# posgraph/coupe.DVSG

Hardware: AMD Instinct MI355X
Metric: stabilized frames/sec (1280x720 RGB) (higher is better)
Workload: dtype f32

## Files before the change

### coupe/dvsg_amd/csrc/cnn_kernels.h

```cpp
#pragma once
#include <type_traits>

#include "common.h"

namespace dvsg {

enum Precision { kF32 = 0, kF16 = 1, kF32S = 2, kF32X = 3 };
inline size_t elem_size(int prec) { return prec == kF16 ? 2 : 4; }

struct ConvGemm {
  int prec;
  const void *x;
  const void *wt;
  const float *bias;
  const void *res;
  void *y;
  int B, H, W, Cin, Ho, Wo, Cout;
  int ksize, stride, pad;
  int res_H, res_W, res_stride;
  int relu;
  int ldx = 0, res_ld = 0, relu_from = -1;
  const void *wt_packed = nullptr;
  const void *wt_packed_a = nullptr;
  const void *wt_packed_h = nullptr;
// ... 12 lines not shown
extern int g_last_conv_kernel[kConvKernelFields];
inline void record_conv_kernel(int family, int a0 = -1, int a1 = -1, int a2 = -1, int a3 = -1, int wsrc = -1) {
  const int rec[kConvKernelFields] = {family, a0, a1, a2, a3, wsrc};
  for (int i = 0; i < kConvKernelFields; ++i) g_last_conv_kernel[i] = rec[i];
}
inline void reset_conv_kernel() { record_conv_kernel(-1); }
template <typename F>
void with_relu_res(bool relu, int res, F &&f) {
  auto with_res = [&](auto relu_c) {
    if (res == 0) f(relu_c, std::integral_constant<int, 0>{});
    else if (res == 1) f(relu_c, std::integral_constant<int, 1>{});
    else f(relu_c, std::integral_constant<int, 2>{});
  };
  if (relu) with_res(std::true_type{});
  else with_res(std::false_type{});
}
inline size_t x3_packed_bytes(int rows, int K) { return (size_t)rows * K * 6; }
int launch_pack_x3(const float *wt, void *out, int rows, int K, hipStream_t s);
int launch_conv_wide16(const ConvGemm &p, hipStream_t s);
size_t wide16_packed_bytes(int rows, int Cin, int ksize);
int launch_pack_wide16(const void *wt, void *out, int rows, int Cin, int ksize, int order, hipStream_t s);
int launch_zero_tickets(int *tickets, size_t n, hipStream_t s);
struct ConvFused {
  const float *x;
  const float *wt2;
  const float *bias2;
  const float *wt3;
  const float *bias3;
  const float *res;
  float *y;
  int B, H, W, Cin, Ho, Wo, Cout;
  int stride;
  int res_H, res_W, res_stride;
  const float *sc_x = nullptr;
  const float *sc_wt = nullptr;
  const float *sc_bias = nullptr;
  int sc_cin = 0;
  int pieces = 0;
  int f16 = 0;
  int x3 = 0;
};
int launch_conv3x3_1x1_x3(const ConvFused &p, hipStream_t s);
bool conv_fusable(int prec, int Cin, int Cmid, int Cout, int ksize);
int launch_conv3x3_1x1(const ConvFused &p, hipStream_t s);

constexpr int kConv1Cin = 21;
constexpr int kConv1K = 7 * kConv1Cin;
constexpr int kConv1Kpad = 148;
constexpr int kConv1Ld = 150;
constexpr int kConv1LdH = 168;
constexpr int kConv1X3Ld = 88;
constexpr int kConv1X3StageElems = 3 * 64 * kConv1X3Ld;
constexpr int kRootMaxFrames = 16;
constexpr int rootconv_pitch(int cin) { return cin | 1; }
constexpr int rootconv_kpad(int cin) { return (7 * rootconv_pitch(cin) + 3) & ~3; }
constexpr int rootconv_ld(int cin) { return rootconv_kpad(cin) + 2; }
constexpr int kRootKernelFields = 9;
enum RootKernelField { kRootConv1 = 0, kRootNW, kRootTO, kRootSRC, kRootBands, kRootQuads, kRootMaxpool, kRootAvgpool,
                       kRootDenseChunks };
extern int g_last_root_kernel[kRootKernelFields];
inline void reset_root_kernel() {
  for (int i = 0; i < kRootKernelFields; ++i) g_last_root_kernel[i] = -1;
}
inline void record_conv1_kernel(int family, int nw, int to, int src, int bands = -1, int quads = -1) {
  const int rec[6] = {family, nw, to, src, bands, quads};
  for (int i = 0; i < 6; ++i) g_last_root_kernel[i] = rec[i];
}
enum Conv1SrcKind { kSrcWindow = 0, kSrcRingF32 = 1, kSrcRingU8 = 2 };
constexpr int kSrcAligned = 1;
constexpr int kSrcKindShift = 1;
constexpr int kSrcMasked = 8;
constexpr int conv1_src(int kind, bool aligned, bool masked) {
  return (kind << kSrcKindShift) | (aligned ? kSrcAligned : 0) | (masked ? kSrcMasked : 0);
}
struct Conv1Src {
  const void *base;
  const int *table;
  int n_pool;
  const float *mask = nullptr;
};
int launch_conv1(int out_prec, const Conv1Src &src, int src_kind, const float *wt1, const void *wt1h, const void *wt1s,
                 const void *wt1x, const float *bias, void *y, int B, int H, int W, int Ho, int Wo, int cin, hipStream_t s);
int prepare_rootconv();

int launch_maxpool(int prec, const void *x, void *y, int B, int H, int W, int C, int Ho, int Wo, int pad_top,
                   int pad_left, hipStream_t s);

constexpr int kPoolSplits = 8;
int launch_avgpool_partial(int prec, const void *x, float *part, int B, int HW, int C, hipStream_t s);

int launch_f16_to_f32(const void *x, float *y, size_t n, hipStream_t s);
int launch_p_to_f32(const void *x, float *y, size_t n, hipStream_t s);
int launch_f32_to_p(const float *x, void *y, size_t n, hipStream_t s);

constexpr int kDenseSplits = 8;
int launch_dense(const float *xin, int s_in, const float *bias_in, float scale_in, int lrelu_in,
                 const float *W, float *out_part, int B, int K, int N, hipStream_t s);
int launch_dense_finalize(const float *part, int s_in, float scale, const float *bias, float *out, int B,
                          int N, hipStream_t s);

}
```

### coupe/dvsg_amd/csrc/conv1_pool.hip

```cpp
#include <cstdint>
#include <type_traits>
#include <utility>

#include "cnn_device.h"
#include "cnn_kernels.h"

namespace dvsg {
namespace {

constexpr int C1_TILE = 128;
constexpr int C1_SEG_PAD = 5488;
constexpr int C1_WELEMS = 64 * kConv1Ld;
constexpr int C1_LDC = 68;

template <int NT, int GROUPS, bool ALIGNED, bool MASKED = false>
struct Conv1Row {
  static constexpr bool kRing = false;
  typedef float floatx4_u __attribute__((ext_vector_type(4), aligned(4)));
  floatx4 nmean[GROUPS];
  long idx[GROUPS];
  unsigned col_ok, full;
  bool fast;
  struct Data {
    floatx4 reg[GROUPS];
// ... 376 lines not shown
#pragma unroll
    for (int q = 0; q < 16; ++q) acc[mi][q] = acc2[mi][q] = 0.f;

#ifdef DVSG_STAMPS
  unsigned long long st[8] = {0, 0, 0, 0, 0, 0, 0, 0};
  const unsigned long long t_begin = C1_STAMP(), r_begin = __builtin_amdgcn_s_memrealtime();
#endif
  load_stage(0);
#ifdef DVSG_STAMPS
  st[0] = C1_STAMP() - t_begin;
#endif
  for (int kh = 0; kh < 7; ++kh) {
#ifdef DVSG_STAMPS
    const unsigned long long s0 = C1_STAMP();
    __syncthreads();
    const unsigned long long s1 = C1_STAMP();
    store_stage();
    const unsigned long long s2 = C1_STAMP();
    __syncthreads();
    const unsigned long long s3 = C1_STAMP();
    if (kh + 1 < 7) load_stage(kh + 1);
    const unsigned long long s4 = C1_STAMP();
    st[1] += s1 - s0;
    st[2] += s2 - s1;
    st[3] += s3 - s2;
    st[4] += s4 - s3;
#else
    __syncthreads();
    store_stage();
    __syncthreads();
    if (kh + 1 < 7) load_stage(kh + 1);
#endif
    __builtin_amdgcn_sched_barrier(0);
    const float *a0 = in_s + 2 * kConv1Cin * (wm * 32 * MI + r) + 2 * h;
    const float *bp = w_s + (wn * 32 + r) * kConv1Ld + 2 * h;
    constexpr int STEPS = kConv1Kpad / 4, PAIRS = (STEPS + 1) / 2;
    float2 va[2][2][MI], vb[2][2];
    auto read_pair = [&](int slot, int g) __attribute__((always_inline)) {
#pragma unroll
      for (int j = 0; j < 2; ++j) {
        if (2 * g + j >= STEPS) break;
#pragma unroll
        for (int mi = 0; mi < MI; ++mi)
          va[slot][j][mi] = *reinterpret_cast<const float2 *>(a0 + mi * (2 * kConv1Cin * 32) + 4 * (2 * g + j));
        vb[slot][j] = *reinterpret_cast<const float2 *>(bp + 4 * (2 * g + j));
      }
    };
    read_pair(0, 0);
#pragma unroll
    for (int g = 0; g < PAIRS; ++g) {
      if (g + 1 < PAIRS) read_pair((g + 1) & 1, g + 1);
      __builtin_amdgcn_sched_barrier(0);
#pragma unroll
      for (int j = 0; j < 2; ++j) {
        if (2 * g + j >= STEPS) break;
#pragma unroll
        for (int mi = 0; mi < MI; ++mi) acc[mi] = mfma32(va[g & 1][j][mi].x, vb[g & 1][j].x, acc[mi]);
#pragma unroll
        for (int mi = 0; mi < MI; ++mi) acc2[mi] = mfma32(va[g & 1][j][mi].y, vb[g & 1][j].y, acc2[mi]);
      }
      __builtin_amdgcn_sched_barrier(0);
    }
  }

#ifdef DVSG_STAMPS
  const unsigned long long t_loop_end = C1_STAMP();
#endif
  float *Cs = w_s;
  __syncthreads();
#pragma unroll
  for (int mi = 0; mi < MI; ++mi)
    C1_TILE_PUT(Cs, wm * 32 * MI + mi * 32, wn * 32, acc[mi][q] + acc2[mi][q]);
  __syncthreads();
  TO *yrow = y + (((size_t)b * Ho + ho) * Wo + wo0) * 64 + 4 * (tid & 15);
  conv1_tile_out<NT / 16>(Cs, conv1_tile_bias(bias, tid), tid, wo0, Wo,
                          [&](int row, float4 v) __attribute__((always_inline)) { store4(yrow + (size_t)row * 64, v); });
#ifdef DVSG_STAMPS
  if (tid == 0 && blockIdx.x < 65536) {
    unsigned long long *o = g_c1_stamps + (size_t)blockIdx.x * 8;
    const unsigned long long t_end = C1_STAMP();
    o[0] = st[0]; o[1] = st[1]; o[2] = st[2]; o[3] = st[3]; o[4] = st[4];
    o[5] = t_loop_end - t_begin;
    o[6] = t_end - t_begin;
    o[7] = __builtin_amdgcn_s_memrealtime() - r_begin;
  }
#endif
}

struct PPieces {};

constexpr int rootconv_seg(int cin) { return C1_RING_PX * rootconv_pitch(cin) + 4; }
constexpr int rootconv_wstage(int cin) { return 64 * rootconv_ld(cin) > C1_TILE * C1_LDC ? 64 * rootconv_ld(cin) : C1_TILE * C1_LDC; }
constexpr size_t rootconv_lds_bytes(int cin) { return sizeof(float) * (size_t)(rootconv_wstage(cin) + rootconv_seg(cin)); }
static_assert(rootconv_lds_bytes(3 * kRootMaxFrames) <= 160 * 1024, "the largest window must fit one workgroup's LDS");

template <typename TO, int SRC>
__global__ __launch_bounds__(256)
void rootconv_kernel(const Conv1Src src, const float *__restrict__ wt1, const float *__restrict__ bias, void *__restrict__ y,
                     int H, int W, int Ho, int Wo, int wtiles, int cin) {
  constexpr int NT = 256, MI = 2;
  constexpr int kKind = SRC >> kSrcKindShift & 3;
  constexpr bool kMasked = (SRC & kSrcMasked) != 0;
  static_assert(SRC >= 0 && SRC < 16 && kKind <= kSrcRingU8, "no such conv1 source");
  extern __shared__ __attribute__((aligned(16))) float rc_lds[];
  const int S = cin / 3, pitch = rootconv_pitch(cin), ldw = rootconv_ld(cin), steps = rootconv_kpad(cin) / 4;
  const int welems = 64 * ldw, seg = rootconv_seg(cin);
  float *w_s = rc_lds;
  float *in_s = rc_lds + rootconv_wstage(cin);
  const int tid = threadIdx.x;
  const int lane = tid & 63, wave = tid >> 6;
  const int wm = wave >> 1, wn = wave & 1;
  const int r = lane & 31, h = lane >> 5;

  const Conv1Tile tile = conv1_tile(wtiles, Ho);
  const int b = tile.b, ho = tile.ho, wo0 = tile.wo0;

  for (int e = tid; e < seg; e += NT) in_s[e] = 0.f;

  const float *mplane = nullptr;
  if constexpr (kMasked) mplane = src.mask + (size_t)b * H * W;
  const int items = C1_RING_PX * S;
  auto stage = [&](int kh) __attribute__((always_inline)) {
    const int hi = 2 * ho + kh - 3;
    const bool row_ok = hi >= 0 && hi < H;
    for (int q = tid; q < items; q += NT) {
      const int f = q / C1_RING_PX, p = q - f * C1_RING_PX;
      const int col = 2 * wo0 - 3 + p;
      float a[3] = {0.f, 0.f, 0.f};
      if (row_ok && col >= 0 && col < W) {
        const size_t px = (size_t)hi * W + col;
        float m = 1.0f;
        bool masked = false;
        if constexpr (kMasked) {
          masked = f < S - 1;
          if (masked) m = mplane[px];
        }
        float s3[3];
        if constexpr (kKind == kSrcWindow) {
          const float *x = static_cast<const float *>(src.base) + ((size_t)b * H * W + px) * cin + 3 * f;
#pragma unroll
          for (int j = 0; j < 3; ++j) s3[j] = masked ? (x[j] * m) * 255.0f : x[j] * 255.0f;
        } else {
          const int fi = src.table[b * S + f];
          const bool frame_ok = fi >= 0 && fi < src.n_pool;
          const size_t e0 = ((size_t)(frame_ok ? fi : 0) * H * W + px) * 3;
          if constexpr (kKind == kSrcRingU8) {
            const uint8_t *x = static_cast<const uint8_t *>(src.base) + e0;
#pragma unroll
            for (int j = 0; j < 3; ++j) {
              const float v = (float)x[j];
              if (masked) {
                const float q0 = v * (1.0f / 255.0f);
                const float xf = __builtin_fmaf(__builtin_fmaf(-q0, 255.0f, v), 1.0f / 255.0f, q0);
                s3[j] = (xf * m) * 255.0f;
              } else {
                s3[j] = v;
              }
            }
          } else {
            const float *x = static_cast<const float *>(src.base) + e0;
#pragma unroll
            for (int j = 0; j < 3; ++j) s3[j] = masked ? (x[j] * m) * 255.0f : x[j] * 255.0f;
          }
          if (!frame_ok) s3[0] = s3[1] = s3[2] = 0.f;
        }
#pragma unroll
// ... 926 lines not shown
    constexpr bool PIPE = SRC < 2;
    Frag fr[PIPE ? 2 : 1];
    if (PIPE) read_a(fr[0], 0);
#pragma unroll
    for (int t = 0; t < 5; ++t) {
      bf16x8 bw[3][2];
#pragma unroll
      for (int p = 0; p < 3; ++p)
#pragma unroll
        for (int ni = 0; ni < 2; ++ni)
          bw[p][ni] = *reinterpret_cast<const bf16x8 *>(b0 + (p * 64 + ni * 32) * kConv1X3Ld + 16 * t);
      if (PIPE) {
        if (t + 1 < 5) read_a(fr[(t + 1) & 1], t + 1);
      } else {
        read_a(fr[0], t);
      }
      __builtin_amdgcn_sched_barrier(0);
      const Frag &f = fr[PIPE ? (t & 1) : 0];
#define DVSG_C1X_TERM(C, PA, PB) \
  _Pragma("unroll") for (int ni = 0; ni < 2; ++ni) C[ni] = __builtin_amdgcn_mfma_f32_32x32x16_bf16(f.a[PA].v, bw[PB][ni], C[ni], 0, 0, 0)
      DVSG_C1X_TERM(accs, 2, 0);
      DVSG_C1X_TERM(accs, 0, 2);
      DVSG_C1X_TERM(accs, 1, 1);
      DVSG_C1X_TERM(accs, 1, 0);
      DVSG_C1X_TERM(accs, 0, 1);
      DVSG_C1X_TERM(acc, 0, 0);
#undef DVSG_C1X_TERM
      __builtin_amdgcn_sched_barrier(0);
    }
  }

  float *Cs = reinterpret_cast<float *>(w_s);
  __syncthreads();
#pragma unroll
  for (int ni = 0; ni < 2; ++ni)
    C1_TILE_PUT(Cs, wave * 32, ni * 32, acc[ni][q] + accs[ni][q]);
  __syncthreads();
  const int col4 = tid & 15;
  conv1_tile_out<16>(Cs, conv1_tile_bias(bias, tid), tid, wo0, Wo, [&](int row, float4 v) __attribute__((always_inline)) {
    store4(y + (((size_t)b * Ho + ho) * Wo + wo0 + row) * 64 + 4 * col4, v);
  });
}

__global__ __launch_bounds__(256) void maxpool_p_kernel(const void *__restrict__ x, void *__restrict__ y, int H, int W,
                                                       int C4, int Ho, int Wo, int pad_top, int pad_left, size_t total) {
  const size_t e = (size_t)xcd_remap(blockIdx.x, gridDim.x) * 256 + threadIdx.x;
  if (e >= total) return;
  const int c4 = (int)(e % C4);
  size_t t = e / C4;
  const int wo = (int)(t % Wo);
  t /= Wo;
  const int ho = (int)(t % Ho);
  const size_t b = t / Ho;
  float4 m = make_float4(-INFINITY, -INFINITY, -INFINITY, -INFINITY);
#pragma unroll
  for (int i = 0; i < 3; ++i) {
    const int hi = 2 * ho - pad_top + i;
    if (hi < 0 || hi >= H) continue;
#pragma unroll
    for (int j = 0; j < 3; ++j) {
      const int wi = 2 * wo - pad_left + j;
      if (wi < 0 || wi >= W) continue;
      const float4 v = load4_p(x, (((b * H + hi) * W + wi) * C4 + c4) * 4);
      m.x = fmaxf(m.x, v.x);
      m.y = fmaxf(m.y, v.y);
      m.z = fmaxf(m.z, v.z);
      m.w = fmaxf(m.w, v.w);
    }
  }
  store4_p(y, e * 4, m);
}

int march_bands(int B, int Ho, int wtiles, int *quads_per_band) {
  const int quads = (Ho + C1M_QUAD - 1) / C1M_QUAD;
  const long cols = (long)B * wtiles;
  for (int qpb = 8; qpb >= 4; --qpb) {
    const int bands = (quads + qpb - 1) / qpb;
    if (cols * bands >= 3 * 256) {
      if (quads_per_band) *quads_per_band = qpb;
      return bands;
    }
  }
  return 0;
}

template <int S>
using SrcC = std::integral_constant<int, S>;
template <bool MASKED_TOO, typename F>
bool with_conv1_src(int src, F &&f) {
  auto is = [&](auto c) { return src == c && (f(c), true); };
  if (is(SrcC<conv1_src(kSrcWindow, false, false)>{}) || is(SrcC<conv1_src(kSrcWindow, true, false)>{}) ||
      is(SrcC<conv1_src(kSrcRingF32, false, false)>{}) || is(SrcC<conv1_src(kSrcRingF32, true, false)>{}) ||
      is(SrcC<conv1_src(kSrcRingU8, false, false)>{}) || is(SrcC<conv1_src(kSrcRingU8, true, false)>{}))
    return true;
  if constexpr (MASKED_TOO)
    return is(SrcC<conv1_src(kSrcWindow, false, true)>{}) || is(SrcC<conv1_src(kSrcWindow, true, true)>{}) ||
           is(SrcC<conv1_src(kSrcRingF32, false, true)>{}) || is(SrcC<conv1_src(kSrcRingF32, true, true)>{}) ||
           is(SrcC<conv1_src(kSrcRingU8, false, true)>{}) || is(SrcC<conv1_src(kSrcRingU8, true, true)>{});
  return false;
}

}

int g_last_root_kernel[kRootKernelFields] = {-1, -1, -1, -1, -1, -1, -1, -1, -1};

int launch_conv1(int out_prec, const Conv1Src &src, int src_kind, const float *wt1, const void *wt1h, const void *wt1s,
                 const void *wt1x, const float *bias, void *y, int B, int H, int W, int Ho, int Wo, int cin, hipStream_t s) {
  DVSG_REQUIRE(cin % 3 == 0 && cin >= 3 && cin <= 3 * kRootMaxFrames, "conv1: %d input channels", cin);
  const int wtiles = ceil_div(Wo, C1_TILE);
  const long blocks = (long)wtiles * Ho * B;
  DVSG_REQUIRE(blocks > 0 && blocks < (1L << 31), "conv1: grid of %ld workgroups out of range", blocks);
  DVSG_REQUIRE((long)W * cin < (1L << 31), "conv1: input row too long");
  DVSG_REQUIRE(src_kind == kSrcWindow || (src.table && src.n_pool > 0), "conv1: a frame ring needs its index table");
  const double in_bytes = src_kind == kSrcRingU8 ? 1.0 : 4.0;
  ProfScope prof(kClsConv1, s, 2.0 * (double)B * Ho * Wo * 64 * 49 * cin,
                 in_bytes * (double)B * H * W * cin + (double)elem_size(out_prec) * B * Ho * Wo * 64);
  const dim3 grid((unsigned)blocks);
  const bool aligned = W % 4 == 0 && reinterpret_cast<uintptr_t>(src.base) % (src_kind == kSrcRingU8 ? 4 : 16) == 0;
  const int SRC = conv1_src(src_kind, aligned, src.mask != nullptr);
  if (cin != kConv1Cin) {
    DVSG_REQUIRE(wt1, "conv1: no float32 weight image");
    const int to = out_prec == kF16 ? 1 : (out_prec == kF32S ? 2 : 0);
    const size_t lds = rootconv_lds_bytes(cin);
    const bool known = with_conv1_src<true>(SRC, [&](auto src_c) {
      constexpr int S = decltype(src_c)::value;
      record_conv1_kernel(6, 4, to, S);
      if (to == 1)
        hipLaunchKernelGGL((rootconv_kernel<_Float16, S>), grid, dim3(256), lds, s, src, wt1, bias, y, H, W, Ho, Wo, wtiles, cin);
      else if (to == 2)
        hipLaunchKernelGGL((rootconv_kernel<PPieces, S>), grid, dim3(256), lds, s, src, wt1, bias, y, H, W, Ho, Wo, wtiles, cin);
      else
        hipLaunchKernelGGL((rootconv_kernel<float, S>), grid, dim3(256), lds, s, src, wt1, bias, y, H, W, Ho, Wo, wtiles, cin);
    });
    DVSG_REQUIRE(known, "conv1: no kernel for source %d", SRC);
    return check_launch("rootconv_kernel");
  }
  if (out_prec == kF32S && !wt1s) return fail(DVSG_ERR_UNSUPPORTED, "conv1: the f32s precision needs the piece weights");
  if (out_prec == kF32X && !wt1x) return fail(DVSG_ERR_UNSUPPORTED, "conv1: the f32x3 precision needs the bfloat16 piece weights");
  const int variant = g_opt.conv1_variant;
  bool legal = true;
  if (out_prec == kF32X) {
    legal = with_conv1_src<true>(SRC, [&](auto src_c) {
      constexpr int S = decltype(src_c)::value;
      record_conv1_kernel(5, -1, -1, S);
      hipLaunchKernelGGL((conv1_x3_kernel<S>), grid, dim3(256), 0, s, src, static_cast<const unsigned short *>(wt1x), bias,
                         static_cast<float *>(y), H, W, Ho, Wo, wtiles);
    });
  } else if (out_prec == kF32S) {
    legal = with_conv1_src<true>(SRC, [&](auto src_c) {
      constexpr int S = decltype(src_c)::value;
      record_conv1_kernel(4, -1, 0, S);
      hipLaunchKernelGGL((conv1_split_kernel<float, S>), grid, dim3(256), 0, s, src, static_cast<const _Float16 *>(wt1s), bias,
                         static_cast<float *>(y), H, W, Ho, Wo, wtiles);
    });
  } else if (out_prec == kF16 && wt1h && variant == 3 && !src.mask) {
    legal = with_conv1_src<false>(SRC, [&](auto src_c) {
      constexpr int S = decltype(src_c)::value;
      record_conv1_kernel(1, -1, 1, S);
      hipLaunchKernelGGL((conv1_f16_kernel<_Float16, S>), grid, dim3(256), 0, s, src, static_cast<const _Float16 *>(wt1h), bias,
                         static_cast<_Float16 *>(y), H, W, Ho, Wo, wtiles);
    });
  } else if (out_prec == kF16 && wt1h && variant != 2 && variant != 4 && !src.mask &&
             (variant == 5 || march_bands(B, Ho, wtiles, nullptr) > 0)) {
    int qpb = 0;
    int bands = march_bands(B, Ho, wtiles, &qpb);
    if (variant == 5) {
      qpb = 3;
      bands = ((Ho + C1M_QUAD - 1) / C1M_QUAD + qpb - 1) / qpb;
    }
    const dim3 mgrid((unsigned)((long)wtiles * bands * B));
    legal = with_conv1_src<false>(SRC, [&](auto src_c) {
      constexpr int S = decltype(src_c)::value;
      record_conv1_kernel(3, -1, -1, S, bands, qpb);
      hipLaunchKernelGGL((conv1_f16_march_kernel<S>), mgrid, dim3(512), 0, s, src, static_cast<const _Float16 *>(wt1h), bias,
                         static_cast<_Float16 *>(y), H, W, Ho, Wo, wtiles, bands, qpb);
    });
  } else if (out_prec == kF16 && wt1h && variant != 2) {
    const int hpairs = (Ho + 1) / 2;
    const dim3 pgrid((unsigned)((long)wtiles * hpairs * B));
    legal = with_conv1_src<true>(SRC, [&](auto src_c) {
      constexpr int S = decltype(src_c)::value;
      record_conv1_kernel(2, -1, 1, S);
      hipLaunchKernelGGL((conv1_f16_pair_kernel<_Float16, S>), pgrid, dim3(256), 0, s, src, static_cast<const _Float16 *>(wt1h), bias,
                         static_cast<_Float16 *>(y), H, W, Ho, Wo, wtiles, hpairs);
    });
  } else if (out_prec == kF16) {
    DVSG_REQUIRE(src_kind == kSrcWindow && !src.mask, "conv1: conv1_variant 2 takes an unmasked window tensor");
    record_conv1_kernel(0, 4, 1, 0);
    hipLaunchKernelGGL((conv1_kernel<4, _Float16, 0>), grid, dim3(256), 0, s, src, wt1, bias, static_cast<_Float16 *>(y), H, W,
                       Ho, Wo, wtiles);
  } else if (variant != 0 && src_kind == kSrcWindow && !src.mask) {
    record_conv1_kernel(0, 8, 0, 0);
    hipLaunchKernelGGL((conv1_kernel<8, float, 0>), grid, dim3(512), 0, s, src, wt1, bias, static_cast<float *>(y), H, W, Ho,
                       Wo, wtiles);
  } else {
    legal = with_conv1_src<true>(SRC, [&](auto src_c) {
      constexpr int S = decltype(src_c)::value;
      record_conv1_kernel(0, 4, 0, S);
      hipLaunchKernelGGL((conv1_kernel<4, float, S>), grid, dim3(256), 0, s, src, wt1, bias, static_cast<float *>(y), H, W, Ho, Wo,
                         wtiles);
    });
  }
  DVSG_REQUIRE(legal, "conv1: no kernel for source %d", SRC);
  return check_launch("conv1_kernel");
}

int prepare_rootconv() {
  const int bytes = (int)rootconv_lds_bytes(3 * kRootMaxFrames);
  hipError_t err = hipSuccess;
  auto raise = [&](const void *fn) {
    const hipError_t e = hipFuncSetAttribute(fn, hipFuncAttributeMaxDynamicSharedMemorySize, bytes);
    if (err == hipSuccess) err = e;
  };
  for (int src = 0; src < 16; ++src)
    with_conv1_src<true>(src, [&](auto src_c) {
      constexpr int S = decltype(src_c)::value;
      raise(reinterpret_cast<const void *>(&rootconv_kernel<float, S>));
      raise(reinterpret_cast<const void *>(&rootconv_kernel<_Float16, S>));
      raise(reinterpret_cast<const void *>(&rootconv_kernel<PPieces, S>));
    });
  DVSG_HIP(err);
  return DVSG_OK;
}

#ifdef DVSG_STAMPS
extern "C" int dvsg_debug_read_conv1_stamps(void *host, size_t bytes) {
  return hipMemcpyFromSymbol(host, HIP_SYMBOL(g_c1_stamps), bytes) == hipSuccess ? 0 : -3;
}
#endif

int launch_maxpool(int prec, const void *x, void *y, int B, int H, int W, int C, int Ho, int Wo, int pad_top,
                   int pad_left, hipStream_t s) {
  DVSG_REQUIRE(C % 4 == 0 && (prec != kF32S || C % 32 == 0), "maxpool: C=%d must be a multiple of 4 (32 in the f32s format)", C);
  const size_t total = (size_t)B * Ho * Wo * (C / 4);
  const size_t want = (total + 255) / 256;
  DVSG_REQUIRE(want < (1u << 31), "maxpool: %zu blocks do not fit a grid", want);
  const int blocks = (int)want;
  ProfScope prof(kClsMaxpool, s, 0.0, (double)elem_size(prec) * C * ((double)B * H * W + (double)B * Ho * Wo));
  g_last_root_kernel[kRootMaxpool] = prec == kF32S ? 3 : (prec == kF16 ? (C % 8 == 0 ? 2 : 1) : 0);
  if (prec == kF32S)
    hipLaunchKernelGGL(maxpool_p_kernel, dim3(blocks), dim3(256), 0, s, x, y, H, W, C / 4, Ho, Wo, pad_top, pad_left, total);
  else if (prec == kF16 && C % 8 == 0) {
    const size_t total8 = total / 2;
    hipLaunchKernelGGL(maxpool_h8_kernel, dim3((unsigned)((total8 + 255) / 256)), dim3(256), 0, s, static_cast<const _Float16 *>(x),
                       static_cast<_Float16 *>(y), H, W, C / 8, Ho, Wo, pad_top, pad_left, total8);
  } else if (prec == kF16)
    hipLaunchKernelGGL(maxpool_kernel<_Float16>, dim3(blocks), dim3(256), 0, s, static_cast<const _Float16 *>(x),
                       static_cast<_Float16 *>(y), H, W, C / 4, Ho, Wo, pad_top, pad_left, total);
  else
    hipLaunchKernelGGL(maxpool_kernel<float>, dim3(blocks), dim3(256), 0, s, static_cast<const float *>(x),
                       static_cast<float *>(y), H, W, C / 4, Ho, Wo, pad_top, pad_left, total);
  return check_launch("maxpool_kernel");
}

}
```

### coupe/dvsg_amd/csrc/locnet.hip

```cpp
#include <cmath>
#include <cstring>
#include <map>
#include <string>
#include <vector>

#include "cnn_kernels.h"

namespace dvsg {
namespace {

constexpr float kBnEps = 1e-5f;
const char *kPrefix = "stabNet/localizationNet/";

struct HostArray {
  const float *data;
  int nd;
  int64_t dims[4];
  size_t size() const {
    size_t n = 1;
    for (int i = 0; i < nd; ++i) n *= (size_t)dims[i];
    return n;
  }
};

// ... 683 lines not shown
  f.f16 = prec == kF16;
  f.x3 = prec == kF32X;
  f.x = static_cast<const float *>(x); f.wt2 = static_cast<const float *>(wt2); f.bias2 = bias2;
  f.wt3 = static_cast<const float *>(wt3); f.bias3 = bias3;
  f.res = static_cast<const float *>(res); f.y = static_cast<float *>(y);
  f.B = B; f.H = H; f.W = W; f.Cin = Cin; f.Cout = Cout;
  f.Ho = (H - 1) / stride + 1; f.Wo = (W - 1) / stride + 1;
  f.stride = stride;
  f.res_H = (f.Ho - 1) * res_stride + 1; f.res_W = (f.Wo - 1) * res_stride + 1; f.res_stride = res_stride;
  if (sc_x) {
    f.res = nullptr;
    f.sc_x = static_cast<const float *>(sc_x); f.sc_wt = static_cast<const float *>(sc_wt); f.sc_bias = sc_bias;
    f.sc_cin = sc_cin;
  }
  return launch_conv3x3_1x1(f, as_stream(stream));
}

int opt_any(int v) { return v; }
int opt_flag(int v) { return v != 0; }
int opt_positive(int v) { return v > 0 ? v : 1; }
int opt_mask16(int v) { return v & 0xFFFF; }
constexpr struct {
  const char *name;
  int DebugOptions::*member;
  int (*normalise)(int);
} kDebugOptions[] = {
    {"conv_variant", &DebugOptions::conv_variant, opt_any},
    {"conv1_variant", &DebugOptions::conv1_variant, opt_any},
    {"wide16_min_tiles", &DebugOptions::wide16_min_tiles, opt_any},
    {"wide16_packed", &DebugOptions::wide16_packed, opt_any},
    {"wide16_arows", &DebugOptions::wide16_arows, opt_any},
    {"wide16_hreuse", &DebugOptions::wide16_hreuse, opt_any},
    {"fused_hreuse", &DebugOptions::fused_hreuse, opt_any},
    {"fuse_conv", &DebugOptions::fuse_conv, opt_any},
    {"fuse_shortcut", &DebugOptions::fuse_shortcut, opt_flag},
    {"concat_sc", &DebugOptions::concat_sc, opt_flag},
    {"x3_conv1", &DebugOptions::x3_conv1, opt_any},
    {"x3_fuse", &DebugOptions::x3_fuse, opt_any},
    {"f16_split", &DebugOptions::f16_split, opt_flag},
    {"f16_pair_mask", &DebugOptions::f16_pair_mask, opt_mask16},
    {"flow_tiled", &DebugOptions::flow_tiled, opt_any},
    {"flow_rounds", &DebugOptions::flow_rounds, opt_positive},
    {"warp_xcd", &DebugOptions::warp_xcd, opt_flag},
};

}
}

extern "C" {

int dvsg_locnet_create(int n_arrays, const char *const *names, const float *const *host_data, const int *ndims,
                       const int64_t *dims, dvsg_locnet_t **out) {
  DVSG_REQUIRE(names && host_data && ndims && dims && out && n_arrays > 0, "dvsg_locnet_create: bad arguments");
  *out = nullptr;
  ArrayMap m;
  for (int i = 0; i < n_arrays; ++i) {
    DVSG_REQUIRE(names[i] && host_data[i] && ndims[i] >= 1 && ndims[i] <= 4, "dvsg_locnet_create: bad array %d", i);
    std::string name(names[i]);
    if (name.size() > 2 && name.compare(name.size() - 2, 2, ":0") == 0) name.resize(name.size() - 2);
    HostArray a;
    a.data = host_data[i];
    a.nd = ndims[i];
    for (int j = 0; j < 4; ++j) a.dims[j] = j < a.nd ? dims[(size_t)i * 4 + j] : 1;
    m[name] = a;
  }
  const std::string rn = std::string(kPrefix) + "resnet_v1_50";
  auto it = m.find(rn + "/conv1/weights");
  if (it == m.end()) return fail(DVSG_ERR_WEIGHTS, "checkpoint array missing: %s/conv1/weights", rn.c_str());
  if (it->second.nd != 4) return fail(DVSG_ERR_WEIGHTS, "conv1/weights must be 4-D");
  const int c_in = (int)it->second.dims[2];
  if (c_in < 3 || c_in > 3 * kRootMaxFrames || c_in % 3 != 0)
    return fail(DVSG_ERR_UNSUPPORTED, "conv1 has %d input channels; this build supports windows of S RGB frames, c_in = 3 S, S <= %d",
                c_in, kRootMaxFrames);

  dvsg_locnet *net = new dvsg_locnet();
  net->c_in = c_in;
  int rc = DVSG_OK;
  auto bail = [&](int code) {
    dvsg_locnet_destroy(net);
    return code;
  };
  net->conv1 = ConvLayer{7, c_in, 64, 2, true};
  if ((rc = make_conv1(net, m, rn + "/conv1", &net->conv1))) return bail(rc);
  if (c_in != kConv1Cin && (rc = prepare_rootconv())) return bail(rc);
  int depth_in = 64;
  for (const BlockSpec &bs : kBlocks) {
    for (int u = 1; u <= bs.units; ++u) {
      Unit unit;
      unit.block = (int)(&bs - kBlocks);
      unit.base = bs.base;
      unit.depth = bs.base * 4;
      unit.stride = u == bs.units ? bs.last_stride : 1;
      unit.has_shortcut = depth_in != unit.depth;
      const std::string sc = rn + "/" + bs.name + "/unit_" + std::to_string(u) + "/bottleneck_v1";
      if (unit.has_shortcut) {
        if (unit.stride != 1) return bail(fail(DVSG_ERR_UNSUPPORTED, "strided shortcut conv not expected in resnet_v1_50"));
        unit.shortcut = ConvLayer{1, depth_in, unit.depth, 1, false};
        if ((rc = make_conv(net, m, sc + "/shortcut", &unit.shortcut))) return bail(rc);
      }
      unit.c1 = ConvLayer{1, depth_in, bs.base, 1, true};
      unit.c2 = ConvLayer{3, bs.base, bs.base, unit.stride, true};
      unit.c3 = ConvLayer{1, bs.base, unit.depth, 1, false};
      if ((rc = make_conv(net, m, sc + "/conv1", &unit.c1))) return bail(rc);
      if ((rc = make_conv(net, m, sc + "/conv2", &unit.c2))) return bail(rc);
      if ((rc = make_conv(net, m, sc + "/conv3", &unit.c3))) return bail(rc);
      if (unit.has_shortcut && unit.shortcut.cin % 64 == 0 && unit.shortcut.cin > 64) {
        const ConvLayer &a = unit.shortcut, &b = unit.c1;
        unit.cat = ConvLayer{1, a.cin, a.cout + b.cout, 1, false};
        const size_t ka = (size_t)a.cout * a.cin, kb = (size_t)b.cout * b.cin;
        void *w = nullptr, *ws2 = nullptr, *bi = nullptr, *w3 = nullptr;
        if (hipMalloc(&w, (ka + kb) * sizeof(float)) != hipSuccess || hipMalloc(&ws2, 2 * (ka + kb) * sizeof(_Float16)) != hipSuccess ||
            hipMalloc(&bi, (a.cout + b.cout) * sizeof(float)) != hipSuccess || hipMalloc(&w3, 6 * (ka + kb)) != hipSuccess)
          return bail(fail(DVSG_ERR_HIP, "hipMalloc failed"));
        net->allocs.push_back(w); net->allocs.push_back(ws2); net->allocs.push_back(bi); net->allocs.push_back(w3);
        hipError_t e = hipMemcpy(w, a.wt, ka * sizeof(float), hipMemcpyDeviceToDevice);
        if (e == hipSuccess) e = hipMemcpy(static_cast<float *>(w) + ka, b.wt, kb * sizeof(float), hipMemcpyDeviceToDevice);
        if (e == hipSuccess) e = hipMemcpy(ws2, a.wt32s, 2 * ka * sizeof(_Float16), hipMemcpyDeviceToDevice);
        if (e == hipSuccess) e = hipMemcpy(static_cast<_Float16 *>(ws2) + 2 * ka, b.wt32s, 2 * kb * sizeof(_Float16), hipMemcpyDeviceToDevice);
        if (e == hipSuccess) e = hipMemcpy(w3, a.wt3x, 6 * ka, hipMemcpyDeviceToDevice);
        if (e == hipSuccess) e = hipMemcpy(static_cast<char *>(w3) + 6 * ka, b.wt3x, 6 * kb, hipMemcpyDeviceToDevice);
        if (e == hipSuccess) e = hipMemcpy(bi, a.bias, a.cout * sizeof(float), hipMemcpyDeviceToDevice);
        if (e == hipSuccess) e = hipMemcpy(static_cast<float *>(bi) + a.cout, b.bias, b.cout * sizeof(float), hipMemcpyDeviceToDevice);
        if (e != hipSuccess) return bail(fail(DVSG_ERR_HIP, "concatenating shortcut | conv1: %s", hipGetErrorString(e)));
        unit.cat.wt = static_cast<float *>(w);
        unit.cat.wt32s = static_cast<_Float16 *>(ws2);
        unit.cat.wt3x = static_cast<unsigned short *>(w3);
        unit.cat.bias = static_cast<float *>(bi);
        unit.has_cat = true;
      }
      net->units.push_back(unit);
      depth_in = unit.depth;
    }
  }
  for (int i = 0; i < 4; ++i) {
    const std::string sc = std::string(kPrefix) + "df/dense" + std::to_string(i + 1);
    const HostArray *W, *b;
    if ((rc = find(m, sc + "/W", {kDenseDims[i][0], kDenseDims[i][1]}, &W))) return bail(rc);
    if ((rc = find(m, sc + "/b", {kDenseDims[i][1]}, &b))) return bail(rc);
    std::vector<float> hw(W->data, W->data + W->size()), hb(b->data, b->data + b->size());
    if ((rc = upload(net, hw, &net->dense_w[i]))) return bail(rc);
    if ((rc = upload(net, hb, &net->dense_b[i]))) return bail(rc);
  }
  std::vector<float> vs(50);
  for (int i = 0; i < 5; ++i)
    for (int j = 0; j < 5; ++j) {
      vs[(i * 5 + j) * 2 + 0] = -1.0f + 0.5f * j;
      vs[(i * 5 + j) * 2 + 1] = -1.0f + 0.5f * i;
    }
  if ((rc = upload(net, vs, &net->v_src))) return bail(rc);
  {
    void *w = nullptr, *scratch = nullptr;
    if (hipMalloc(&w, 25 * 28 * sizeof(double)) != hipSuccess) return bail(fail(DVSG_ERR_HIP, "hipMalloc failed"));
    net->allocs.push_back(w);
    if (hipMalloc(&scratch, 13 * 25 * 2 * sizeof(float)) != hipSuccess) return bail(fail(DVSG_ERR_HIP, "hipMalloc failed"));
    rc = tps_inverse_columns(net->v_src, 25, static_cast<double *>(w), static_cast<float *>(scratch), nullptr);
    (void)hipFree(scratch);
    if (rc) return bail(rc);
    net->winv = static_cast<double *>(w);
  }
  *out = net;
  return DVSG_OK;
}

int dvsg_locnet_destroy(dvsg_locnet_t *net) {
  if (!net) return DVSG_OK;
  for (void *p : net->allocs) (void)hipFree(p);
  delete net;
// ... 448 lines not shown
```

Measured before the change: 743.2.

## Add band-persistent conv1 kernel reusing input rows across output row pairs

Adds a root_band_kernel where each block walks a band of output row pairs. It keeps a 3-slot ring of input rows in LDS and double-buffers the weights per kernel row, so overlapping input rows are loaded once instead of per output row. The next pair's rows and weights are prefetched while the epilogue runs. A host heuristic picks the band count to fill the GPU over a few rounds, and the path becomes the default f32 conv1 path whenever that heuristic finds a valid band count. The trade-off is fewer blocks, heavy LDS use and more synchronisation.

```diff
diff --git a/coupe/dvsg_amd/csrc/cnn_kernels.h b/coupe/dvsg_amd/csrc/cnn_kernels.h
--- a/coupe/dvsg_amd/csrc/cnn_kernels.h
+++ b/coupe/dvsg_amd/csrc/cnn_kernels.h
@@ -118,6 +118,7 @@
 int launch_conv1(int out_prec, const Conv1Src &src, int src_kind, const float *wt1, const void *wt1h, const void *wt1s,
                  const void *wt1x, const float *bias, void *y, int B, int H, int W, int Ho, int Wo, int cin, hipStream_t s);
 int prepare_rootconv();
+int prepare_root_band();
 
 int launch_maxpool(int prec, const void *x, void *y, int B, int H, int W, int C, int Ho, int Wo, int pad_top,
                    int pad_left, hipStream_t s);
diff --git a/coupe/dvsg_amd/csrc/conv1_pool.hip b/coupe/dvsg_amd/csrc/conv1_pool.hip
--- a/coupe/dvsg_amd/csrc/conv1_pool.hip
+++ b/coupe/dvsg_amd/csrc/conv1_pool.hip
@@ -482,6 +482,211 @@
     o[0] = st[0]; o[1] = st[1]; o[2] = st[2]; o[3] = st[3]; o[4] = st[4];
     o[5] = t_loop_end - t_begin;
     o[6] = t_end - t_begin;
+    o[7] = __builtin_amdgcn_s_memrealtime() - r_begin;
+  }
+#endif
+}
+
+constexpr int RB_NT = 512;
+constexpr int RB_IN4 = (C1_SEG_PAD / 4 + RB_NT - 1) / RB_NT;
+constexpr int RB_WLOADS = (C1_WELEMS / 4 + RB_NT - 1) / RB_NT;
+constexpr int RB_SLOTS = 3;
+constexpr size_t RB_LDS = sizeof(float) * (size_t)(2 * C1_WELEMS + RB_SLOTS * C1_SEG_PAD);
+static_assert(RB_LDS <= 160 * 1024, "the band kernel's LDS must fit a CU");
+
+template <int SRC>
+__global__ __launch_bounds__(RB_NT) __attribute__((amdgpu_waves_per_eu(2, 2)))
+void root_band_kernel(const Conv1Src src, const float *__restrict__ wt1, const float *__restrict__ bias,
+                      float *__restrict__ y, int H, int W, int Ho, int Wo, int wtiles, int bands, int ppb, int nbig) {
+  constexpr int NT = RB_NT, MI = 2;
+  static_assert(C1_TILE * C1_LDC <= C1_WELEMS, "epilogue tile must fit in a weight buffer");
+  extern __shared__ __attribute__((aligned(16))) float rb_lds[];
+  float *const w_s = rb_lds;
+  float *const in_s = rb_lds + 2 * C1_WELEMS;
+  const int tid = threadIdx.x;
+  const int lane = tid & 63, wave = tid >> 6;
+  const int wr = wave >> 2, wm = (wave >> 1) & 1, wn = wave & 1;
+  const int r = lane & 31, h = lane >> 5;
+
+  const Conv1Tile tile = conv1_tile(wtiles, bands);
+  const int b = tile.b, band = tile.ho, wo0 = tile.wo0;
+  const int pairs = (Ho + 1) / 2;
+  const int p0 = band * ppb - (band > nbig ? band - nbig : 0);
+  const int p1 = min(p0 + (band < nbig ? ppb : ppb - 1), pairs);
+  if (p0 >= p1) return;
+
+#ifdef DVSG_STAMPS
+  unsigned long long st[8] = {0, 0, 0, 0, 0, 0, 0, 0};
+  const unsigned long long t_begin = C1_STAMP(), r_begin = __builtin_amdgcn_s_memrealtime();
+#endif
+  typedef typename Conv1RowSel<NT, RB_IN4, SRC>::type Row;
+  Row row;
+  row.init(src, tid, b, wo0, H, W, C1_SEG_PAD);
+  if constexpr (Row::kRing) {
+    for (int e = tid; e < RB_SLOTS * C1_SEG_PAD; e += NT) in_s[e] = 0.f;
+    __syncthreads();
+  }
+  typename Row::Data rd[3];
+  floatx4 w_reg[RB_WLOADS];
+  auto load_w = [&](int kh) __attribute__((always_inline)) {
+    const floatx4 *wsrc = reinterpret_cast<const floatx4 *>(wt1 + (size_t)kh * C1_WELEMS);
+#pragma unroll
+    for (int i = 0; i < RB_WLOADS; ++i) {
+      const int q = tid + NT * i;
+      w_reg[i] = wsrc[q < C1_WELEMS / 4 ? q : 0];
+    }
+  };
+  auto put_w = [&](int i, float *dst) __attribute__((always_inline)) {
+    const int q = tid + NT * i;
+    if (q < C1_WELEMS / 4) reinterpret_cast<floatx4 *>(dst)[q] = w_reg[i];
+  };
+  auto put_row = [&](const typename Row::Data &d, float *slot) __attribute__((always_inline)) {
+    if constexpr (Row::kRing) {
+      row.scatter(d, [&](int e, float v) __attribute__((always_inline)) { slot[e] = v; });
+    } else {
+#pragma unroll
+      for (int i = 0; i < RB_IN4; ++i) {
+        const int q = tid + NT * i;
+        const floatx4 v = row.scaled(d, i);
+        if (q < C1_SEG_PAD / 4) reinterpret_cast<floatx4 *>(slot)[q] = v;
+      }
+    }
+  };
+  auto load_first = [&](int ho_) __attribute__((always_inline)) {
+#pragma unroll
+    for (int i = 0; i < 3; ++i) row.load(rd[i], 2 * ho_ - 3 + i);
+    load_w(0);
+  };
+#ifdef DVSG_STAMPS
+  st[0] = C1_STAMP() - t_begin;
+#endif
+  load_first(2 * p0);
+
+  for (int p = p0; p < p1; ++p) {
+    const int ho = 2 * p;
+#ifdef DVSG_STAMPS
+    const unsigned long long f0 = C1_STAMP();
+#endif
+#pragma unroll
+    for (int i = 0; i < RB_WLOADS; ++i) put_w(i, w_s);
+#pragma unroll
+    for (int i = 0; i < 3; ++i) {
+      __builtin_amdgcn_sched_barrier(0);
+      put_row(rd[i], in_s + i * C1_SEG_PAD);
+    }
+    __builtin_amdgcn_sched_barrier(0);
+    floatx16 acc[MI], acc2[MI];
+#pragma unroll
+    for (int mi = 0; mi < MI; ++mi)
+#pragma unroll
+      for (int q = 0; q < 16; ++q) acc[mi][q] = acc2[mi][q] = 0.f;
+#ifdef DVSG_STAMPS
+    const unsigned long long f1 = C1_STAMP();
+    __syncthreads();
+    st[2] += f1 - f0;
+    st[3] += C1_STAMP() - f1;
+#else
+    __syncthreads();
+#endif
+
+    int s_up = 0;
+    for (int t = 0; t < 7; ++t) {
+#ifdef DVSG_STAMPS
+      const unsigned long long s3 = C1_STAMP();
+#endif
+      if (t < 6) {
+        row.load(rd[0], 2 * ho + t);
+        load_w(t + 1);
+      }
+#ifdef DVSG_STAMPS
+      st[4] += C1_STAMP() - s3;
+#endif
+      __builtin_amdgcn_sched_barrier(0);
+      const int s_lo = s_up == 0 ? 2 : s_up - 1;
+      const float *a0 = in_s + (wr ? s_lo : s_up) * C1_SEG_PAD + 2 * kConv1Cin * (wm * 32 * MI + r) + 2 * h;
+      const float *bp = w_s + (t & 1) * C1_WELEMS + (wn * 32 + r) * kConv1Ld + 2 * h;
+      float *w_next = w_s + ((t + 1) & 1) * C1_WELEMS;
+      constexpr int STEPS = kConv1Kpad / 4, PAIRS = (STEPS + 1) / 2;
+      constexpr int WPUT0 = PAIRS / 2;
+      float2 va[2][2][MI], vb[2][2];
+      auto read_pair = [&](int slot, int g) __attribute__((always_inline)) {
+#pragma unroll
+        for (int j = 0; j < 2; ++j) {
+          if (2 * g + j >= STEPS) break;
+#pragma unroll
+          for (int mi = 0; mi < MI; ++mi)
+            va[slot][j][mi] = *reinterpret_cast<const float2 *>(a0 + mi * (2 * kConv1Cin * 32) + 4 * (2 * g + j));
+          vb[slot][j] = *reinterpret_cast<const float2 *>(bp + 4 * (2 * g + j));
+        }
+      };
+      read_pair(0, 0);
+#pragma unroll
+      for (int g = 0; g < PAIRS; ++g) {
+        if (g + 1 < PAIRS) read_pair((g + 1) & 1, g + 1);
+        if (g >= WPUT0 && g < WPUT0 + RB_WLOADS) put_w(g - WPUT0, w_next);
+        __builtin_amdgcn_sched_barrier(0);
+#pragma unroll
+        for (int j = 0; j < 2; ++j) {
+          if (2 * g + j >= STEPS) break;
+#pragma unroll
+          for (int mi = 0; mi < MI; ++mi) acc[mi] = mfma32(va[g & 1][j][mi].x, vb[g & 1][j].x, acc[mi]);
+#pragma unroll
+          for (int mi = 0; mi < MI; ++mi) acc2[mi] = mfma32(va[g & 1][j][mi].y, vb[g & 1][j].y, acc2[mi]);
+        }
+        __builtin_amdgcn_sched_barrier(0);
+      }
+      if (t < 6) {
+#ifdef DVSG_STAMPS
+        const unsigned long long s0 = C1_STAMP();
+        __syncthreads();
+        const unsigned long long s1 = C1_STAMP();
+        put_row(rd[0], in_s + s_up * C1_SEG_PAD);
+        const unsigned long long s2 = C1_STAMP();
+        __syncthreads();
+        st[1] += s1 - s0;
+        st[2] += s2 - s1;
+        st[3] += C1_STAMP() - s2;
+#else
+        __syncthreads();
+        put_row(rd[0], in_s + s_up * C1_SEG_PAD);
+        __syncthreads();
+#endif
+      }
+      s_up = s_up == 2 ? 0 : s_up + 1;
+    }
+
+#ifdef DVSG_STAMPS
+    const unsigned long long e0 = C1_STAMP();
+#endif
+    __syncthreads();
+    float *Cs = w_s + wr * C1_WELEMS;
+#pragma unroll
+    for (int mi = 0; mi < MI; ++mi)
+      C1_TILE_PUT(Cs, wm * 32 * MI + mi * 32, wn * 32, acc[mi][q] + acc2[mi][q]);
+    __builtin_amdgcn_sched_barrier(0);
+    if (p + 1 < p1) load_first(ho + 2);
+    int tid_e = tid;
+    asm volatile("" : "+v"(tid_e));
+    const float4 b4 = conv1_tile_bias(bias, tid_e);
+    __builtin_amdgcn_sched_barrier(0);
+    __syncthreads();
+#pragma unroll
+    for (int j = 0; j < 2; ++j) {
+      if (ho + j >= Ho) break;
+      float *yrow = y + (((size_t)b * Ho + ho + j) * Wo + wo0) * 64 + 4 * (tid_e & 15);
+      conv1_tile_out<NT / 16>(w_s + j * C1_WELEMS, b4, tid_e, wo0, Wo,
+                              [&](int row_, float4 v) __attribute__((always_inline)) { store4(yrow + (size_t)row_ * 64, v); });
+    }
+    __syncthreads();
+#ifdef DVSG_STAMPS
+    st[5] += C1_STAMP() - e0;
+#endif
+  }
+#ifdef DVSG_STAMPS
+  if (tid == 0 && blockIdx.x < 65536) {
+    unsigned long long *o = g_c1_stamps + (size_t)blockIdx.x * 8;
+    o[0] = st[0]; o[1] = st[1]; o[2] = st[2]; o[3] = st[3]; o[4] = st[4]; o[5] = st[5];
+    o[6] = C1_STAMP() - t_begin;
     o[7] = __builtin_amdgcn_s_memrealtime() - r_begin;
   }
 #endif
@@ -1574,6 +1779,28 @@
     }
   }
   return 0;
+}
+
+int root_bands(int B, int Ho, int wtiles, int *pairs_per_band, int *nbig) {
+  const int pairs = (Ho + 1) / 2;
+  const long cols = (long)B * wtiles;
+  int best = 0;
+  double best_fill = 0.0;
+  for (int rounds = 3; rounds <= 6; ++rounds) {
+    const long fit = 256L * rounds / cols, bands = fit < pairs / 4 ? fit : pairs / 4;
+    if (bands < 1 || cols * bands < 3 * 256) continue;
+    const double fill = (double)(cols * bands) / (256.0 * rounds);
+    if (fill > best_fill) {
+      best_fill = fill;
+      best = (int)bands;
+    }
+  }
+  if (best > 0) {
+    const int ppb = (pairs + best - 1) / best;
+    if (pairs_per_band) *pairs_per_band = ppb;
+    if (nbig) *nbig = pairs - best * (ppb - 1);
+  }
+  return best;
 }
 
 template <int S>
@@ -1681,7 +1908,21 @@
     record_conv1_kernel(0, 4, 1, 0);
     hipLaunchKernelGGL((conv1_kernel<4, _Float16, 0>), grid, dim3(256), 0, s, src, wt1, bias, static_cast<_Float16 *>(y), H, W,
                        Ho, Wo, wtiles);
-  } else if (variant != 0 && src_kind == kSrcWindow && !src.mask) {
+  } else if (!src.mask && (variant == 6 || (variant == 0 && root_bands(B, Ho, wtiles, nullptr, nullptr) > 0))) {
+    int ppb = 0, nbig = 0;
+    int bands = root_bands(B, Ho, wtiles, &ppb, &nbig);
+    if (variant == 6) {
+      ppb = 3;
+      bands = nbig = ((Ho + 1) / 2 + ppb - 1) / ppb;
+    }
+    const dim3 bgrid((unsigned)((long)wtiles * bands * B));
+    legal = with_conv1_src<false>(SRC, [&](auto src_c) {
+      constexpr int S = decltype(src_c)::value;
+      record_conv1_kernel(7, 8, 0, S, bands, ppb);
+      hipLaunchKernelGGL((root_band_kernel<S>), bgrid, dim3(RB_NT), RB_LDS, s, src, wt1, bias, static_cast<float *>(y), H, W, Ho,
+                         Wo, wtiles, bands, ppb, nbig);
+    });
+  } else if (variant != 0 && variant != 7 && src_kind == kSrcWindow && !src.mask) {
     record_conv1_kernel(0, 8, 0, 0);
     hipLaunchKernelGGL((conv1_kernel<8, float, 0>), grid, dim3(512), 0, s, src, wt1, bias, static_cast<float *>(y), H, W, Ho,
                        Wo, wtiles);
@@ -1710,6 +1951,19 @@
       raise(reinterpret_cast<const void *>(&rootconv_kernel<float, S>));
       raise(reinterpret_cast<const void *>(&rootconv_kernel<_Float16, S>));
       raise(reinterpret_cast<const void *>(&rootconv_kernel<PPieces, S>));
+    });
+  DVSG_HIP(err);
+  return DVSG_OK;
+}
+
+int prepare_root_band() {
+  hipError_t err = hipSuccess;
+  for (int src = 0; src < 16; ++src)
+    with_conv1_src<false>(src, [&](auto src_c) {
+      constexpr int S = decltype(src_c)::value;
+      const hipError_t e = hipFuncSetAttribute(reinterpret_cast<const void *>(&root_band_kernel<S>),
+                                               hipFuncAttributeMaxDynamicSharedMemorySize, (int)RB_LDS);
+      if (err == hipSuccess) err = e;
     });
   DVSG_HIP(err);
   return DVSG_OK;
diff --git a/coupe/dvsg_amd/csrc/locnet.hip b/coupe/dvsg_amd/csrc/locnet.hip
--- a/coupe/dvsg_amd/csrc/locnet.hip
+++ b/coupe/dvsg_amd/csrc/locnet.hip
@@ -789,7 +789,7 @@
   };
   net->conv1 = ConvLayer{7, c_in, 64, 2, true};
   if ((rc = make_conv1(net, m, rn + "/conv1", &net->conv1))) return bail(rc);
-  if (c_in != kConv1Cin && (rc = prepare_rootconv())) return bail(rc);
+  if ((rc = c_in != kConv1Cin ? prepare_rootconv() : prepare_root_band())) return bail(rc);
   int depth_in = 64;
   for (const BlockSpec &bs : kBlocks) {
     for (int u = 1; u <= bs.units; ++u) {
```

New measurement: 753.3 (median of 6 runs). 1.01x the previous value.
